# Atten4Vis/LW-DETR

Hardware: AMD Instinct MI355X
Metric: images/sec (higher is better)
Workload: dtype fp16; 1 GPU; LW-DETR-small inference forward + PostProcess, 640x640, batch 32/GPU, fp16, random-init weights (synthetic COCO-shaped input); global_batch=32, per_gpu_batch=32, parallelism=dp1, collective=none, launch_chains=2

## Files before the change

### lw-detr_amd/csrc/rowops.hip

```cpp
#include "common.h"

namespace {

constexpr int LN_MAX_CHUNKS = 16;

inline bool aligned16(const void* p) { return ((uintptr_t)p & 15) == 0; }

template <typename T, int NCH>
__global__ __launch_bounds__(256) void layernorm_kernel(const T* x, long ldx, const float* __restrict__ gamma,
                                                        const float* __restrict__ beta, T* out, long ldo,
                                                        long M, int C, float eps, long rows_per_batch,
                                                        long out_batch_rows, long out_row_offset,
                                                        const float* __restrict__ gamma2, const float* __restrict__ beta2,
                                                        T* __restrict__ out2, long ldo2, float eps2,
                                                        const float* __restrict__ part, int nsplit,
                                                        const float* __restrict__ pbias) {
    constexpr int EPC = 16 / (int)sizeof(T);
    typedef T VC __attribute__((ext_vector_type(EPC)));
    const int lane16 = threadIdx.x & 15;
    const long row = (long)blockIdx.x * 16 + (threadIdx.x >> 4);
    if (row >= M) return;
    const int nchunks = C / EPC;
    const T* xr = x + row * ldx;
    float v[NCH][EPC];
    float sum = 0.f;
#pragma unroll
    for (int i = 0; i < NCH; ++i) {
        const int c = lane16 + 16 * i;
        if (c < nchunks) {
            const VC t = *(const VC*)(xr + c * EPC);
#pragma unroll
            for (int e = 0; e < EPC; ++e) v[i][e] = to_f32<T>(t[e]);
            if (part) {
                float a[EPC];
#pragma unroll
                for (int e = 0; e < EPC; ++e) a[e] = pbias[c * EPC + e];
#pragma unroll 4
                for (int sidx = 0; sidx < nsplit; ++sidx) {
                    const float* pr = part + ((long)sidx * M + row) * C + c * EPC;
#pragma unroll
                    for (int e4 = 0; e4 < EPC; e4 += 4) {
                        const f32x4 q = *(const f32x4*)(pr + e4);
                        a[e4] += q[0]; a[e4 + 1] += q[1]; a[e4 + 2] += q[2]; a[e4 + 3] += q[3];
                    }
                }
#pragma unroll
                for (int e = 0; e < EPC; ++e) v[i][e] = to_f32<T>(from_f32<T>(v[i][e] + a[e]));
            }
#pragma unroll
            for (int e = 0; e < EPC; ++e) sum += v[i][e];
        }
    }
#pragma unroll
// ... 160 lines not shown
    hipStream_t st = (hipStream_t)hip_stream;
    switch (dtype) {
        case DT_F32: return launch_row_stats<float>(x, ldx, M, C, eps, stats, st);
        case DT_F16: return launch_row_stats<f16>(x, ldx, M, C, eps, stats, st);
        case DT_BF16: return launch_row_stats<bf16>(x, ldx, M, C, eps, stats, st);
        default: return LWDETR_ERR_UNSUPPORTED;
    }
}

extern "C" int lwdetr_layernorm(const void* x, long ldx, const float* gamma, const float* beta, void* out, long ldo,
                                long M, int C, float eps, long rows_per_batch, long out_batch_rows, long out_row_offset,
                                int dtype, void* hip_stream) {
    if (!x || !gamma || !beta || !out || M < 0 || C <= 0) return LWDETR_ERR_BAD_ARG;
    if (M == 0) return LWDETR_OK;
    hipStream_t st = (hipStream_t)hip_stream;
    switch (dtype) {
        case DT_F32: return launch_ln<float>(x, ldx, gamma, beta, out, ldo, M, C, eps, rows_per_batch, out_batch_rows, out_row_offset, st);
        case DT_F16: return launch_ln<f16>(x, ldx, gamma, beta, out, ldo, M, C, eps, rows_per_batch, out_batch_rows, out_row_offset, st);
        case DT_BF16: return launch_ln<bf16>(x, ldx, gamma, beta, out, ldo, M, C, eps, rows_per_batch, out_batch_rows, out_row_offset, st);
        default: return LWDETR_ERR_UNSUPPORTED;
    }
}

extern "C" int lwdetr_layernorm_chain(const void* x, long ldx, const float* gamma1, const float* beta1, float eps1, void* out1,
                                      long ldo1, const float* gamma2, const float* beta2, float eps2, void* out2, long ldo2,
                                      long M, int C, int dtype, void* hip_stream) {
    if (!x || !gamma1 || !beta1 || !out1 || !gamma2 || !beta2 || !out2 || M < 0 || C <= 0) return LWDETR_ERR_BAD_ARG;
    if (M == 0) return LWDETR_OK;
    hipStream_t st = (hipStream_t)hip_stream;
    switch (dtype) {
        case DT_F32: return launch_ln<float>(x, ldx, gamma1, beta1, out1, ldo1, M, C, eps1, 0, 0, 0, st, gamma2, beta2, out2, ldo2, eps2);
        case DT_F16: return launch_ln<f16>(x, ldx, gamma1, beta1, out1, ldo1, M, C, eps1, 0, 0, 0, st, gamma2, beta2, out2, ldo2, eps2);
        case DT_BF16: return launch_ln<bf16>(x, ldx, gamma1, beta1, out1, ldo1, M, C, eps1, 0, 0, 0, st, gamma2, beta2, out2, ldo2, eps2);
        default: return LWDETR_ERR_UNSUPPORTED;
    }
}

extern "C" int lwdetr_ffn_finish(const void* x, long ldx, const float* partial, int splits, const float* b2, const float* gamma1,
                                 const float* beta1, float eps1, void* out1, long ldo1, const float* gamma2, const float* beta2,
                                 float eps2, void* out2, long ldo2, long M, int C, int dtype, void* hip_stream) {
    if (!x || !partial || splits <= 0 || !b2 || !gamma1 || !beta1 || !out1 || M < 0 || C <= 0 || C % 8 != 0) return LWDETR_ERR_BAD_ARG;
    if (gamma2 && (!beta2 || !out2)) return LWDETR_ERR_BAD_ARG;
    if (M == 0) return LWDETR_OK;
    hipStream_t st = (hipStream_t)hip_stream;
    switch (dtype) {
        case DT_F16: return launch_ln<f16>(x, ldx, gamma1, beta1, out1, ldo1, M, C, eps1, 0, 0, 0, st, gamma2, beta2, out2, ldo2, eps2, partial, splits, b2);
        case DT_BF16: return launch_ln<bf16>(x, ldx, gamma1, beta1, out1, ldo1, M, C, eps1, 0, 0, 0, st, gamma2, beta2, out2, ldo2, eps2, partial, splits, b2);
        default: return LWDETR_ERR_UNSUPPORTED;
    }
}

namespace {

template <typename T>
__global__ __launch_bounds__(256) void select_gather_kernel(const T* __restrict__ om, const T* __restrict__ enc_cls, long ldc,
                                                            const float* __restrict__ props, const int64_t* __restrict__ idx,
                                                            T* __restrict__ om_sel, T* __restrict__ logits_out,
                                                            float* __restrict__ props_sel, int B, int S, int d, int nq, int ncls) {
    const long row = blockIdx.x;
    const int b = (int)(row / nq);
    const long src = (long)b * S + idx[row];
    for (int c = threadIdx.x; c < d; c += blockDim.x) om_sel[row * d + c] = om[src * d + c];
    for (int c = threadIdx.x; c < ncls; c += blockDim.x) logits_out[row * ncls + c] = enc_cls[src * ldc + c];
    if (threadIdx.x < 4) props_sel[row * 4 + threadIdx.x] = props[src * 4 + threadIdx.x];
}

template <typename T>
__global__ __launch_bounds__(256) void decoder_inputs_kernel(const T* __restrict__ enc_delta, const float* __restrict__ props_sel,
                                                             const float* __restrict__ refpoint, const float* __restrict__ vr,
                                                             int L, const T* __restrict__ query_feat,
                                                             const float* __restrict__ dim_t, T* __restrict__ enc_boxes,
                                                             float* __restrict__ ref_out, T* __restrict__ sine,
                                                             T* __restrict__ xdec, int B, int nq, int d) {
    const long row = blockIdx.x;
    const int b = (int)(row / nq), q = (int)(row - (long)b * nq);
    float dl[4], pr[4], ts[4], rp[4], rf[4];
#pragma unroll
    for (int i = 0; i < 4; ++i) { dl[i] = to_f32<T>(enc_delta[row * 4 + i]); pr[i] = props_sel[row * 4 + i]; rp[i] = refpoint[q * 4 + i]; }
    ts[0] = dl[0] * pr[2] + pr[0]; ts[1] = dl[1] * pr[3] + pr[1]; ts[2] = expf(dl[2]) * pr[2]; ts[3] = expf(dl[3]) * pr[3];
    rf[0] = rp[0] * ts[2] + ts[0]; rf[1] = rp[1] * ts[3] + ts[1]; rf[2] = expf(rp[2]) * ts[2]; rf[3] = expf(rp[3]) * ts[3];
    if (threadIdx.x < 4) { enc_boxes[row * 4 + threadIdx.x] = from_f32<T>(ts[threadIdx.x]); ref_out[row * 4 + threadIdx.x] = rf[threadIdx.x]; }
    const float vx = vr[(long)b * L * 2], vy = vr[(long)b * L * 2 + 1];
    const float pos[4] = {rf[1] * vy, rf[0] * vx, rf[2] * vx, rf[3] * vy};
    const int half = d / 2;
    for (int c = threadIdx.x; c < 2 * d; c += blockDim.x) {
        const int k = c / half, i = c - k * half;
        const float e = pos[k] * 6.283185307179586f / dim_t[i];
        sine[row * 2 * d + c] = from_f32<T>((i & 1) ? __cosf(e) : __sinf(e));
    }
    for (int c = threadIdx.x; c < d; c += blockDim.x) xdec[row * d + c] = query_feat[(long)q * d + c];
}

template <typename T>
__global__ __launch_bounds__(256) void box_reparam_kernel(const T* __restrict__ delta, const float* __restrict__ ref, long ref_rows,
                                                          T* __restrict__ out, long R) {
    const long r = (long)blockIdx.x * blockDim.x + threadIdx.x;
    if (r >= R) return;
    const float* rf = ref + (r % ref_rows) * 4;
    const float d0 = to_f32<T>(delta[r * 4]), d1 = to_f32<T>(delta[r * 4 + 1]), d2 = to_f32<T>(delta[r * 4 + 2]), d3 = to_f32<T>(delta[r * 4 + 3]);
    out[r * 4] = from_f32<T>(d0 * rf[2] + rf[0]);
    out[r * 4 + 1] = from_f32<T>(d1 * rf[3] + rf[1]);
    out[r * 4 + 2] = from_f32<T>(expf(d2) * rf[2]);
    out[r * 4 + 3] = from_f32<T>(expf(d3) * rf[3]);
}

template <typename T>
__global__ __launch_bounds__(256) void finalize_outputs_kernel(const T* __restrict__ delta, const float* __restrict__ ref, long ref_rows,
                                                               T* __restrict__ coord, long R, const T* __restrict__ logits_pad,
                                                               long ldc, int ncls, T* __restrict__ logits_out, long layer_gap) {
    const long i = (long)blockIdx.x * blockDim.x + threadIdx.x;
    if (i < R * ncls) {
        const long r = i / ncls;
        const long orow = r + (r / ref_rows) * layer_gap;
        logits_out[orow * ncls + (i - r * ncls)] = logits_pad[r * ldc + (i - r * ncls)];
    }
    if (i < R) {
        const long k = i % ref_rows;
        const float* rf = ref + k * 4;
        T* o = coord + (i + (i / ref_rows) * layer_gap) * 4;
        const float d0 = to_f32<T>(delta[i * 4]), d1 = to_f32<T>(delta[i * 4 + 1]), d2 = to_f32<T>(delta[i * 4 + 2]), d3 = to_f32<T>(delta[i * 4 + 3]);
        o[0] = from_f32<T>(d0 * rf[2] + rf[0]);
        o[1] = from_f32<T>(d1 * rf[3] + rf[1]);
        o[2] = from_f32<T>(expf(d2) * rf[2]);
        o[3] = from_f32<T>(expf(d3) * rf[3]);
    }
}

}

#define LWDETR_DISPATCH_T(dtype, CALL)                 \
    switch (dtype) {                                   \
        case DT_F32: { typedef float TT; CALL; break; } \
        case DT_F16: { typedef f16 TT; CALL; break; }   \
        case DT_BF16: { typedef bf16 TT; CALL; break; } \
        default: return LWDETR_ERR_UNSUPPORTED;        \
    }

extern "C" int lwdetr_select_gather(const void* om, const void* enc_cls, long ldc, const float* props, const int64_t* idx,
                                    void* om_sel, void* logits_out, float* props_sel, int B, int S, int d, int nq, int ncls,
                                    int dtype, void* hip_stream) {
    if (!om || !enc_cls || !props || !idx || !om_sel || !logits_out || !props_sel || B <= 0 || nq <= 0 || S <= 0 ||
        d <= 0 || ncls <= 0 || ldc < ncls) return LWDETR_ERR_BAD_ARG;
    hipStream_t st = (hipStream_t)hip_stream;
    ProfScope ps(KID_ELTWISE, 0.0, 2.0 * B * nq * (d + ncls) * 2, st);
    LWDETR_DISPATCH_T(dtype, hipLaunchKernelGGL((select_gather_kernel<TT>), dim3(B * nq), dim3(256), 0, st, (const TT*)om,
                                                (const TT*)enc_cls, ldc, props, idx, (TT*)om_sel, (TT*)logits_out, props_sel, B,
                                                S, d, nq, ncls));
    return lwdetr_check_launch();
}

extern "C" int lwdetr_decoder_inputs(const void* enc_delta, const float* props_sel, const float* refpoint, const float* valid_ratios,
                                     int L, const void* query_feat, const float* dim_t, void* enc_boxes_out, float* ref_out,
                                     void* sine_out, void* xdec_out, int B, int nq, int d, int dtype, void* hip_stream) {
    if (!enc_delta || !props_sel || !refpoint || !valid_ratios || !query_feat || !dim_t || !enc_boxes_out || !ref_out ||
        !sine_out || !xdec_out || B <= 0 || nq <= 0 || d <= 0 || d % 2 || L <= 0) return LWDETR_ERR_BAD_ARG;
    hipStream_t st = (hipStream_t)hip_stream;
    ProfScope ps(KID_ELTWISE, 0.0, 3.0 * B * nq * d * 2, st);
    LWDETR_DISPATCH_T(dtype, hipLaunchKernelGGL((decoder_inputs_kernel<TT>), dim3(B * nq), dim3(256), 0, st, (const TT*)enc_delta,
                                                props_sel, refpoint, valid_ratios, L, (const TT*)query_feat, dim_t,
                                                (TT*)enc_boxes_out, ref_out, (TT*)sine_out, (TT*)xdec_out, B, nq, d));
    return lwdetr_check_launch();
}

extern "C" int lwdetr_box_reparam(const void* delta, const float* ref, long ref_rows, void* out, long R, int dtype, void* hip_stream) {
    if (!delta || !ref || !out || R < 0 || ref_rows <= 0) return LWDETR_ERR_BAD_ARG;
    if (R == 0) return LWDETR_OK;
    hipStream_t st = (hipStream_t)hip_stream;
    ProfScope ps(KID_ELTWISE, 0.0, 0.0, st);
    LWDETR_DISPATCH_T(dtype, hipLaunchKernelGGL((box_reparam_kernel<TT>), dim3((unsigned)((R + 255) / 256)), dim3(256), 0, st,
                                                (const TT*)delta, ref, ref_rows, (TT*)out, R));
    return lwdetr_check_launch();
}

extern "C" int lwdetr_finalize_outputs(const void* delta, const float* ref, long ref_rows, void* coord_out, long R,
                                       const void* logits_pad, long ldc, int ncls, void* logits_out, long out_layer_rows, int dtype,
                                       void* hip_stream) {
    if (!delta || !ref || !coord_out || !logits_pad || !logits_out || R < 0 || ref_rows <= 0 || ncls <= 0 || ldc < ncls) return LWDETR_ERR_BAD_ARG;
    if (logits_out == logits_pad) return LWDETR_ERR_BAD_ARG;
    if (out_layer_rows == 0) out_layer_rows = ref_rows;
    if (out_layer_rows < ref_rows) return LWDETR_ERR_BAD_ARG;
    if (R == 0) return LWDETR_OK;
    hipStream_t st = (hipStream_t)hip_stream;
    ProfScope ps(KID_ELTWISE, 0.0, 0.0, st);
    const long n = R * ncls;
    LWDETR_DISPATCH_T(dtype, hipLaunchKernelGGL((finalize_outputs_kernel<TT>), dim3((unsigned)((n + 255) / 256)), dim3(256), 0, st,
                                                (const TT*)delta, ref, ref_rows, (TT*)coord_out, R, (const TT*)logits_pad, ldc, ncls,
                                                (TT*)logits_out, out_layer_rows - ref_rows));
    return lwdetr_check_launch();
}
```

### lw-detr_amd/csrc/topk.hip

```cpp
#include "common.h"

namespace {

constexpr int TK_THREADS = 1024;
constexpr int TK_MAXK = 1024;
constexpr int TK_IDX_BITS = 20;
constexpr unsigned TK_IDX_MASK = (1u << TK_IDX_BITS) - 1;

__device__ __forceinline__ unsigned fkey(float f) {
    const unsigned u = __float_as_uint(f);
    return (u & 0x80000000u) ? ~u : (u | 0x80000000u);
}
__device__ __forceinline__ float fkey_inv(unsigned k) {
    return __uint_as_float((k & 0x80000000u) ? (k ^ 0x80000000u) : ~k);
}

__device__ __forceinline__ unsigned long long tk_comp(unsigned key, int i) {
    return ((unsigned long long)key << TK_IDX_BITS) | (unsigned long long)(TK_IDX_MASK - (unsigned)i);
}

struct TopkShared {
    unsigned hist[2048];
    unsigned long long sel[TK_MAXK];
    unsigned rank[TK_MAXK];
    unsigned bstar, above, cnt, nsel;
};

template <typename T, bool CACHE>
__device__ void topk_block(const T* __restrict__ x, int N, int K, TopkShared& sh, unsigned* __restrict__ keys) {
    const int tid = threadIdx.x;
    unsigned long long prefix = 0;
    unsigned rem = (unsigned)K;
    unsigned long long thr = 0;
    int top = 32 + TK_IDX_BITS;
    bool first = true;
    while (true) {
        const int bits = top > 30 ? 11 : 10;
        const int shift = top - bits;
        const unsigned nb = 1u << bits;
        for (int i = tid; i < 2048; i += TK_THREADS) sh.hist[i] = 0;
        __syncthreads();
        if (first) {
            int i = tid;
            for (; i + 3 * TK_THREADS < N; i += 4 * TK_THREADS) {
                unsigned k4[4];
#pragma unroll
                for (int u = 0; u < 4; ++u) k4[u] = fkey(to_f32<T>(x[i + u * TK_THREADS]));
#pragma unroll
                for (int u = 0; u < 4; ++u) {
                    if (CACHE) keys[i + u * TK_THREADS] = k4[u];
                    atomicAdd(&sh.hist[k4[u] >> 21], 1u);
                }
            }
            for (; i < N; i += TK_THREADS) {
                const unsigned k = fkey(to_f32<T>(x[i]));
                if (CACHE) keys[i] = k;
                atomicAdd(&sh.hist[k >> 21], 1u);
            }
        } else {
            for (int i = tid; i < N; i += TK_THREADS) {
                const unsigned long long c = tk_comp(CACHE ? keys[i] : fkey(to_f32<T>(x[i])), i);
                if ((c >> top) == prefix) atomicAdd(&sh.hist[(unsigned)(c >> shift) & (nb - 1)], 1u);
            }
        }
        first = false;
        __syncthreads();
        if (tid < 64) {
            const int per = (int)nb >> 6;
            unsigned own = 0;
            for (int j = 0; j < per; ++j) own += sh.hist[tid * per + ((j + tid) & (per - 1))];
            unsigned s = own;
#pragma unroll
            for (int o = 1; o < 64; o <<= 1) {
                const unsigned t = __shfl_down(s, o);
                if (tid + o < 64) s += t;
            }
            const unsigned excl = s - own;
            if (excl < rem && rem <= s) {
                unsigned acc = excl;
                for (int j = per - 1; j >= 0; --j) {
                    const unsigned c = sh.hist[tid * per + j];
                    if (acc + c >= rem) { sh.bstar = (unsigned)(tid * per + j); sh.above = acc; sh.cnt = c; break; }
                    acc += c;
                }
            }
        }
        __syncthreads();
        const unsigned bstar = sh.bstar, above = sh.above, cnt = sh.cnt;
        rem -= above;
        prefix = (prefix << bits) | bstar;
        top = shift;
        if (cnt == rem || top == 0) { thr = prefix << top; break; }
    }
    if (tid == 0) sh.nsel = 0;
    for (int i = tid; i < TK_MAXK; i += TK_THREADS) sh.rank[i] = 0;
    __syncthreads();
    for (int i = tid; i < N; i += TK_THREADS) {
        const unsigned long long c = tk_comp(CACHE ? keys[i] : fkey(to_f32<T>(x[i])), i);
        if (c >= thr) {
            const unsigned p = atomicAdd(&sh.nsel, 1u);
            if (p < (unsigned)K) sh.sel[p] = c;
        }
    }
    __syncthreads();
    const int parts = TK_THREADS / K > 0 ? TK_THREADS / K : 1;
    const int e = tid % K, p = tid / K;
    if (p < parts) {
        const unsigned long long mine = sh.sel[e];
        const int j0 = (int)((long)K * p / parts), j1 = (int)((long)K * (p + 1) / parts);
        unsigned r = 0;
        for (int j = j0; j < j1; ++j) r += sh.sel[j] > mine ? 1u : 0u;
        atomicAdd(&sh.rank[e], r);
    }
    __syncthreads();
}

template <typename T, bool CACHE>
__global__ __launch_bounds__(TK_THREADS) void topk_kernel(const T* __restrict__ x, int N, int K, int64_t* __restrict__ idx_out,
                                                          float* __restrict__ val_out) {
    __shared__ TopkShared sh;
    extern __shared__ unsigned tk_keys[];
    const int b = blockIdx.x;
    topk_block<T, CACHE>(x + (long)b * N, N, K, sh, tk_keys);
    const int tid = threadIdx.x;
    if (tid < K) {
        const unsigned long long c = sh.sel[tid];
        const unsigned r = sh.rank[tid];
        idx_out[(long)b * K + r] = (int64_t)(TK_IDX_MASK - (unsigned)(c & TK_IDX_MASK));
        if (val_out) val_out[(long)b * K + r] = fkey_inv((unsigned)(c >> TK_IDX_BITS));
    }
}

template <typename T, bool CACHE>
__global__ __launch_bounds__(TK_THREADS) void postprocess_kernel(const T* __restrict__ logits, const T* __restrict__ boxes,
                                                                 const float* __restrict__ sizes, int nq, int ncls, int K,
                                                                 float* __restrict__ scores, int64_t* __restrict__ labels,
                                                                 float* __restrict__ out_boxes, float* __restrict__ packed) {
    __shared__ TopkShared sh;
    extern __shared__ unsigned tk_keys[];
    const int b = blockIdx.x;
    const int N = nq * ncls;
    topk_block<T, CACHE>(logits + (long)b * N, N, K, sh, tk_keys);
    const int tid = threadIdx.x;
    if (tid < K) {
        const unsigned long long c = sh.sel[tid];
        const long o = (long)b * K + sh.rank[tid];
        const int i = (int)(TK_IDX_MASK - (unsigned)(c & TK_IDX_MASK));
        const int q = i / ncls;
        const float v = fkey_inv((unsigned)(c >> TK_IDX_BITS));
        const float score = to_f32<T>(from_f32<T>(1.f / (1.f + expf(-v))));
        const T* bx = boxes + ((long)b * nq + q) * 4;
        const float cx = to_f32<T>(bx[0]), cy = to_f32<T>(bx[1]);
        const float w = fmaxf(to_f32<T>(bx[2]), 0.f), h = fmaxf(to_f32<T>(bx[3]), 0.f);
        const float ih = sizes[b * 2], iw = sizes[b * 2 + 1];
        const float x0 = to_f32<T>(from_f32<T>(cx - 0.5f * w)) * iw, y0 = to_f32<T>(from_f32<T>(cy - 0.5f * h)) * ih;
        const float x1 = to_f32<T>(from_f32<T>(cx + 0.5f * w)) * iw, y1 = to_f32<T>(from_f32<T>(cy + 0.5f * h)) * ih;
        if (packed) {
            float* pr = packed + o * 6;
            pr[0] = score; pr[1] = (float)(i - q * ncls); pr[2] = x0; pr[3] = y0; pr[4] = x1; pr[5] = y1;
        } else {
            scores[o] = score;
            labels[o] = (int64_t)(i - q * ncls);
            out_boxes[o * 4 + 0] = x0; out_boxes[o * 4 + 1] = y0; out_boxes[o * 4 + 2] = x1; out_boxes[o * 4 + 3] = y1;
        }
    }
}

template <typename T>
__global__ __launch_bounds__(256) void rowmax_kernel(const T* __restrict__ x, long ld, long rows, int ncols, float* __restrict__ out) {
    constexpr int EPC = 4;
    typedef T VC __attribute__((ext_vector_type(EPC)));
    const int lane16 = threadIdx.x & 15;
    const long row = (long)blockIdx.x * 16 + (threadIdx.x >> 4);
    float m = -INFINITY;
    if (row < rows) {
        const T* xr = x + row * ld;
        const int full = ncols / EPC;
        for (int c = lane16; c < full; c += 16) {
            const VC t = *(const VC*)(xr + c * EPC);
#pragma unroll
            for (int e = 0; e < EPC; ++e) m = fmaxf(m, to_f32<T>(t[e]));
        }
        for (int c = full * EPC + lane16; c < ncols; c += 16) m = fmaxf(m, to_f32<T>(xr[c]));
    }
#pragma unroll
    for (int o = 8; o >= 1; o >>= 1) m = fmaxf(m, __shfl_xor(m, o));
    if (row < rows && lane16 == 0) out[row] = m;
}

}

constexpr size_t TK_CACHE_BYTES = 160 * 1024 - sizeof(TopkShared) - 256;
static bool tk_allow_lds(const void* fn) {
    static const void* done[16]; static int ndone = 0;
    for (int i = 0; i < ndone; ++i) if (done[i] == fn) return true;
    if (hipFuncSetAttribute(fn, hipFuncAttributeMaxDynamicSharedMemorySize, (int)TK_CACHE_BYTES) != hipSuccess) return false;
    if (ndone < 16) done[ndone++] = fn;
    return true;
}

#define LWDETR_DISPATCH_T(dtype, CALL)                 \
    switch (dtype) {                                   \
        case DT_F32: { typedef float TT; CALL; break; } \
        case DT_F16: { typedef f16 TT; CALL; break; }   \
        case DT_BF16: { typedef bf16 TT; CALL; break; } \
        default: return LWDETR_ERR_UNSUPPORTED;        \
    }

extern "C" int lwdetr_rowmax(const void* x, long ld, long rows, int ncols, float* out, int dtype, void* hip_stream) {
    if (!x || !out || rows < 0 || ncols <= 0 || ld < ncols) return LWDETR_ERR_BAD_ARG;
    if (rows == 0) return LWDETR_OK;
    if (ld % 4 || ((uintptr_t)x & 15)) return LWDETR_ERR_BAD_ARG;
    hipStream_t st = (hipStream_t)hip_stream;
    ProfScope ps(KID_ELTWISE, 0.0, (double)rows * ncols * (dtype == DT_F32 ? 4 : 2), st);
    LWDETR_DISPATCH_T(dtype, hipLaunchKernelGGL((rowmax_kernel<TT>), dim3((unsigned)((rows + 15) / 16)), dim3(256), 0, st,
                                                (const TT*)x, ld, rows, ncols, out));
    return lwdetr_check_launch();
}

extern "C" int lwdetr_topk(const void* x, int B, int N, int K, int64_t* idx_out, float* val_out, int dtype, void* hip_stream) {
    if (!x || !idx_out || B < 0 || K <= 0 || K > N || K > TK_MAXK || N > (int)TK_IDX_MASK) return LWDETR_ERR_BAD_ARG;
    if (B == 0) return LWDETR_OK;
    hipStream_t st = (hipStream_t)hip_stream;
    ProfScope ps(KID_ELTWISE, 0.0, (double)B * N * (dtype == DT_F32 ? 4 : 2), st);
    const bool cache = (size_t)N * 4 <= TK_CACHE_BYTES;
    LWDETR_DISPATCH_T(dtype, {
        if (cache) {
            if (!tk_allow_lds((const void*)topk_kernel<TT, true>)) return LWDETR_ERR_LAUNCH;
            hipLaunchKernelGGL((topk_kernel<TT, true>), dim3(B), dim3(TK_THREADS), (size_t)N * 4, st, (const TT*)x, N, K, idx_out, val_out);
        } else {
            hipLaunchKernelGGL((topk_kernel<TT, false>), dim3(B), dim3(TK_THREADS), 0, st, (const TT*)x, N, K, idx_out, val_out);
        }
    });
    return lwdetr_check_launch();
}

static int postprocess_impl(const void* logits, const void* boxes, const float* target_sizes, int B, int nq, int ncls, int K,
                                  float* scores, int64_t* labels, float* out_boxes, float* packed, int dtype, void* hip_stream) {
    if (!logits || !boxes || !target_sizes || B < 0 || nq <= 0 || ncls <= 0 || K <= 0 ||
        K > TK_MAXK || (long)nq * ncls > (long)TK_IDX_MASK || K > nq * ncls)
        return LWDETR_ERR_BAD_ARG;
    if (B == 0) return LWDETR_OK;
    hipStream_t st = (hipStream_t)hip_stream;
    ProfScope ps(KID_ELTWISE, 0.0, (double)B * nq * ncls * (dtype == DT_F32 ? 4 : 2), st);
    const size_t kb = (size_t)nq * ncls * 4;
    const bool cache = kb <= TK_CACHE_BYTES;
    LWDETR_DISPATCH_T(dtype, {
        if (cache) {
            if (!tk_allow_lds((const void*)postprocess_kernel<TT, true>)) return LWDETR_ERR_LAUNCH;
            hipLaunchKernelGGL((postprocess_kernel<TT, true>), dim3(B), dim3(TK_THREADS), kb, st, (const TT*)logits, (const TT*)boxes,
                               target_sizes, nq, ncls, K, scores, labels, out_boxes, packed);
        } else {
            hipLaunchKernelGGL((postprocess_kernel<TT, false>), dim3(B), dim3(TK_THREADS), 0, st, (const TT*)logits, (const TT*)boxes,
                               target_sizes, nq, ncls, K, scores, labels, out_boxes, packed);
        }
    });
    return lwdetr_check_launch();
}

extern "C" int lwdetr_postprocess(const void* logits, const void* boxes, const float* target_sizes, int B, int nq, int ncls, int K,
                                  float* scores, int64_t* labels, float* out_boxes, int dtype, void* hip_stream) {
    if (!scores || !labels || !out_boxes) return LWDETR_ERR_BAD_ARG;
    return postprocess_impl(logits, boxes, target_sizes, B, nq, ncls, K, scores, labels, out_boxes, nullptr, dtype, hip_stream);
}

extern "C" int lwdetr_postprocess_packed(const void* logits, const void* boxes, const float* target_sizes, int B, int nq, int ncls,
                                         int K, float* packed, int dtype, void* hip_stream) {
    if (!packed) return LWDETR_ERR_BAD_ARG;
    return postprocess_impl(logits, boxes, target_sizes, B, nq, ncls, K, nullptr, nullptr, nullptr, packed, dtype, hip_stream);
}
```

Measured before the change: 14120 images/sec.

## Rework top-k radix select with range-compressed keys and vectorize decoder glue kernels

Rewrites the block-wide top-k used by two-stage proposal selection and PostProcess. It uses vectorized 16-byte loads, computes key min/max to compress the composite key, adds a candidate queue and suffix-sum histogram, picks a 512-thread variant for small N, and computes output ranks directly. The select_gather and decoder_inputs kernels now process four rows per block with one wavefront per row and 16-byte vector copies, replacing one 256-thread block per row. This targets the latency of the small serial selection kernels and the low-utilization glue kernels, at the cost of much more complex top-k code and extra LDS use. Optional timing instrumentation is included but compiled out by default.

Result: faster. 14370 images/sec, median of 6 (+1.8%).

```diff
diff --git a/lw-detr_amd/csrc/rowops.hip b/lw-detr_amd/csrc/rowops.hip
--- a/lw-detr_amd/csrc/rowops.hip
+++ b/lw-detr_amd/csrc/rowops.hip
@@ -1,4 +1,5 @@
 #include "common.h"
+#include <type_traits>
 
 namespace {
 
@@ -265,43 +266,87 @@
 
 namespace {
 
-template <typename T>
+constexpr int GLUE_ROWS = 4;
+
+template <typename T, bool VEC>
 __global__ __launch_bounds__(256) void select_gather_kernel(const T* __restrict__ om, const T* __restrict__ enc_cls, long ldc,
                                                             const float* __restrict__ props, const int64_t* __restrict__ idx,
                                                             T* __restrict__ om_sel, T* __restrict__ logits_out,
-                                                            float* __restrict__ props_sel, int B, int S, int d, int nq, int ncls) {
-    const long row = blockIdx.x;
+                                                            float* __restrict__ props_sel, long rows, int S, int d, int nq, int ncls) {
+    typedef typename Vec<T>::v8 V8;
+    typedef typename Vec<T>::v4 V4;
+    typedef typename std::conditional<sizeof(T) == 2, V8, V4>::type V;
+    constexpr int EPV = 16 / (int)sizeof(T);
+    const int lane = threadIdx.x & 63;
+    const long row = (long)blockIdx.x * GLUE_ROWS + (threadIdx.x >> 6);
+    if (row >= rows) return;
     const int b = (int)(row / nq);
     const long src = (long)b * S + idx[row];
-    for (int c = threadIdx.x; c < d; c += blockDim.x) om_sel[row * d + c] = om[src * d + c];
-    for (int c = threadIdx.x; c < ncls; c += blockDim.x) logits_out[row * ncls + c] = enc_cls[src * ldc + c];
-    if (threadIdx.x < 4) props_sel[row * 4 + threadIdx.x] = props[src * 4 + threadIdx.x];
-}
-
-template <typename T>
+    if (VEC) {
+        const V* __restrict__ sv = (const V*)(om + src * d);
+        V* __restrict__ ov = (V*)(om_sel + row * d);
+        for (int c = lane; c < d / EPV; c += 64) ov[c] = sv[c];
+    } else {
+        for (int c = lane; c < d; c += 64) om_sel[row * d + c] = om[src * d + c];
+    }
+    for (int c = lane; c < ncls; c += 64) logits_out[row * ncls + c] = enc_cls[src * ldc + c];
+    if (lane < 4) props_sel[row * 4 + lane] = props[src * 4 + lane];
+}
+
+template <typename T, bool VEC>
 __global__ __launch_bounds__(256) void decoder_inputs_kernel(const T* __restrict__ enc_delta, const float* __restrict__ props_sel,
                                                              const float* __restrict__ refpoint, const float* __restrict__ vr,
                                                              int L, const T* __restrict__ query_feat,
                                                              const float* __restrict__ dim_t, T* __restrict__ enc_boxes,
                                                              float* __restrict__ ref_out, T* __restrict__ sine,
-                                                             T* __restrict__ xdec, int B, int nq, int d) {
-    const long row = blockIdx.x;
+                                                             T* __restrict__ xdec, long rows, int nq, int d) {
+    typedef typename Vec<T>::v8 V8;
+    typedef typename Vec<T>::v4 V4;
+    typedef typename std::conditional<sizeof(T) == 2, V8, V4>::type V;
+    constexpr int EPV = 16 / (int)sizeof(T);
+    const int lane = threadIdx.x & 63;
+    const long row = (long)blockIdx.x * GLUE_ROWS + (threadIdx.x >> 6);
+    if (row >= rows) return;
     const int b = (int)(row / nq), q = (int)(row - (long)b * nq);
     float dl[4], pr[4], ts[4], rp[4], rf[4];
 #pragma unroll
     for (int i = 0; i < 4; ++i) { dl[i] = to_f32<T>(enc_delta[row * 4 + i]); pr[i] = props_sel[row * 4 + i]; rp[i] = refpoint[q * 4 + i]; }
     ts[0] = dl[0] * pr[2] + pr[0]; ts[1] = dl[1] * pr[3] + pr[1]; ts[2] = expf(dl[2]) * pr[2]; ts[3] = expf(dl[3]) * pr[3];
     rf[0] = rp[0] * ts[2] + ts[0]; rf[1] = rp[1] * ts[3] + ts[1]; rf[2] = expf(rp[2]) * ts[2]; rf[3] = expf(rp[3]) * ts[3];
-    if (threadIdx.x < 4) { enc_boxes[row * 4 + threadIdx.x] = from_f32<T>(ts[threadIdx.x]); ref_out[row * 4 + threadIdx.x] = rf[threadIdx.x]; }
+    if (lane < 4) {
+        const float t = lane == 0 ? ts[0] : lane == 1 ? ts[1] : lane == 2 ? ts[2] : ts[3];
+        const float r = lane == 0 ? rf[0] : lane == 1 ? rf[1] : lane == 2 ? rf[2] : rf[3];
+        enc_boxes[row * 4 + lane] = from_f32<T>(t);
+        ref_out[row * 4 + lane] = r;
+    }
     const float vx = vr[(long)b * L * 2], vy = vr[(long)b * L * 2 + 1];
-    const float pos[4] = {rf[1] * vy, rf[0] * vx, rf[2] * vx, rf[3] * vy};
+    const float p0 = rf[1] * vy, p1 = rf[0] * vx, p2 = rf[2] * vx, p3 = rf[3] * vy;
     const int half = d / 2;
-    for (int c = threadIdx.x; c < 2 * d; c += blockDim.x) {
-        const int k = c / half, i = c - k * half;
-        const float e = pos[k] * 6.283185307179586f / dim_t[i];
-        sine[row * 2 * d + c] = from_f32<T>((i & 1) ? __cosf(e) : __sinf(e));
-    }
-    for (int c = threadIdx.x; c < d; c += blockDim.x) xdec[row * d + c] = query_feat[(long)q * d + c];
+    if (VEC) {
+        V* __restrict__ sv = (V*)(sine + row * 2 * d);
+        for (int ch = lane; ch < 2 * d / EPV; ch += 64) {
+            const int c0 = ch * EPV, k = c0 / half, i0 = c0 - k * half;
+            const float pk = k == 0 ? p0 : k == 1 ? p1 : k == 2 ? p2 : p3;
+            V o;
+#pragma unroll
+            for (int u = 0; u < EPV; ++u) {
+                const float e = pk * 6.283185307179586f / dim_t[i0 + u];
+                o[u] = from_f32<T>((u & 1) ? __cosf(e) : __sinf(e));
+            }
+            sv[ch] = o;
+        }
+        const V* __restrict__ qv = (const V*)(query_feat + (long)q * d);
+        V* __restrict__ xv = (V*)(xdec + row * d);
+        for (int c = lane; c < d / EPV; c += 64) xv[c] = qv[c];
+    } else {
+        for (int c = lane; c < 2 * d; c += 64) {
+            const int k = c / half, i = c - k * half;
+            const float pk = k == 0 ? p0 : k == 1 ? p1 : k == 2 ? p2 : p3;
+            const float e = pk * 6.283185307179586f / dim_t[i];
+            sine[row * 2 * d + c] = from_f32<T>((i & 1) ? __cosf(e) : __sinf(e));
+        }
+        for (int c = lane; c < d; c += 64) xdec[row * d + c] = query_feat[(long)q * d + c];
+    }
 }
 
 template <typename T>
@@ -356,9 +401,15 @@
         d <= 0 || ncls <= 0 || ldc < ncls) return LWDETR_ERR_BAD_ARG;
     hipStream_t st = (hipStream_t)hip_stream;
     ProfScope ps(KID_ELTWISE, 0.0, 2.0 * B * nq * (d + ncls) * 2, st);
-    LWDETR_DISPATCH_T(dtype, hipLaunchKernelGGL((select_gather_kernel<TT>), dim3(B * nq), dim3(256), 0, st, (const TT*)om,
-                                                (const TT*)enc_cls, ldc, props, idx, (TT*)om_sel, (TT*)logits_out, props_sel, B,
-                                                S, d, nq, ncls));
+    const long rows = (long)B * nq;
+    const dim3 grid((unsigned)((rows + GLUE_ROWS - 1) / GLUE_ROWS));
+    const int epv = dtype == DT_F32 ? 4 : 8;
+    const bool vec = d % epv == 0 && !(((uintptr_t)om | (uintptr_t)om_sel) & 15);
+#define GLUE_LAUNCH(VEC)                                                                                                          \
+    hipLaunchKernelGGL((select_gather_kernel<TT, VEC>), grid, dim3(64 * GLUE_ROWS), 0, st, (const TT*)om, (const TT*)enc_cls, ldc, \
+                       props, idx, (TT*)om_sel, (TT*)logits_out, props_sel, rows, S, d, nq, ncls)
+    LWDETR_DISPATCH_T(dtype, { if (vec) GLUE_LAUNCH(true); else GLUE_LAUNCH(false); });
+#undef GLUE_LAUNCH
     return lwdetr_check_launch();
 }
 
@@ -369,9 +420,16 @@
         !sine_out || !xdec_out || B <= 0 || nq <= 0 || d <= 0 || d % 2 || L <= 0) return LWDETR_ERR_BAD_ARG;
     hipStream_t st = (hipStream_t)hip_stream;
     ProfScope ps(KID_ELTWISE, 0.0, 3.0 * B * nq * d * 2, st);
-    LWDETR_DISPATCH_T(dtype, hipLaunchKernelGGL((decoder_inputs_kernel<TT>), dim3(B * nq), dim3(256), 0, st, (const TT*)enc_delta,
-                                                props_sel, refpoint, valid_ratios, L, (const TT*)query_feat, dim_t,
-                                                (TT*)enc_boxes_out, ref_out, (TT*)sine_out, (TT*)xdec_out, B, nq, d));
+    const long rows = (long)B * nq;
+    const dim3 grid((unsigned)((rows + GLUE_ROWS - 1) / GLUE_ROWS));
+    const int epv = dtype == DT_F32 ? 4 : 8;
+    const bool vec = (d / 2) % epv == 0 && !(((uintptr_t)query_feat | (uintptr_t)sine_out | (uintptr_t)xdec_out) & 15);
+#define GLUE_LAUNCH(VEC)                                                                                                               \
+    hipLaunchKernelGGL((decoder_inputs_kernel<TT, VEC>), grid, dim3(64 * GLUE_ROWS), 0, st, (const TT*)enc_delta, props_sel, refpoint, \
+                       valid_ratios, L, (const TT*)query_feat, dim_t, (TT*)enc_boxes_out, ref_out, (TT*)sine_out, (TT*)xdec_out, rows, \
+                       nq, d)
+    LWDETR_DISPATCH_T(dtype, { if (vec) GLUE_LAUNCH(true); else GLUE_LAUNCH(false); });
+#undef GLUE_LAUNCH
     return lwdetr_check_launch();
 }
 
diff --git a/lw-detr_amd/csrc/topk.hip b/lw-detr_amd/csrc/topk.hip
--- a/lw-detr_amd/csrc/topk.hip
+++ b/lw-detr_amd/csrc/topk.hip
@@ -1,11 +1,27 @@
 #include "common.h"
+#include <type_traits>
+
+#ifdef LWDETR_TK_TIMING
+__device__ unsigned long long g_tk_timing[16];
+#define TK_TS(i) do { if (blockIdx.x == 0 && threadIdx.x == 0) g_tk_timing[i] = __builtin_amdgcn_s_memrealtime(); } while (0)
+extern "C" int lwdetr_debug_tk_timing(unsigned long long* out) {
+    return hipMemcpyFromSymbol(out, HIP_SYMBOL(g_tk_timing), sizeof(g_tk_timing)) == hipSuccess ? 0 : 1;
+}
+#else
+#define TK_TS(i) do {} while (0)
+#endif
 
 namespace {
 
-constexpr int TK_THREADS = 1024;
 constexpr int TK_MAXK = 1024;
 constexpr int TK_IDX_BITS = 20;
 constexpr unsigned TK_IDX_MASK = (1u << TK_IDX_BITS) - 1;
+constexpr int TK_BINS = 2048;
+constexpr int TK_DIGIT = 11;
+constexpr int TK_QUEUE = 128;
+constexpr int TK_CAND = 512;
+constexpr int TK_SMALL_THREADS = 512, TK_LARGE_THREADS = 1024;
+constexpr int TK_SMALL_N = 4096;
 
 __device__ __forceinline__ unsigned fkey(float f) {
     const unsigned u = __float_as_uint(f);
@@ -15,144 +31,362 @@
     return __uint_as_float((k & 0x80000000u) ? (k ^ 0x80000000u) : ~k);
 }
 
-__device__ __forceinline__ unsigned long long tk_comp(unsigned key, int i) {
-    return ((unsigned long long)key << TK_IDX_BITS) | (unsigned long long)(TK_IDX_MASK - (unsigned)i);
-}
-
-struct TopkShared {
-    unsigned hist[2048];
+template <typename T> struct TkVec { typedef typename Vec<T>::v8 type; };
+template <> struct TkVec<float> { typedef f32x4 type; };
+
+struct alignas(32) TopkShared {
+    unsigned hist[TK_BINS];
+    unsigned sfx[TK_BINS];
     unsigned long long sel[TK_MAXK];
-    unsigned rank[TK_MAXK];
+    unsigned long long cand[TK_CAND];
+    unsigned long long queue[16][TK_QUEUE];
+    unsigned wtot[16], wmin[16], wmax[16];
     unsigned bstar, above, cnt, nsel;
 };
 
-template <typename T, bool CACHE>
-__device__ void topk_block(const T* __restrict__ x, int N, int K, TopkShared& sh, unsigned* __restrict__ keys) {
+struct TkCode {
+    unsigned kmin, idxmask, bstar1;
+    int nb, sh1;
+    __device__ __forceinline__ unsigned long long comp(unsigned key, int i) const {
+        return ((unsigned long long)(key - kmin) << nb) | (unsigned long long)(idxmask - (unsigned)i);
+    }
+    __device__ __forceinline__ int index(unsigned long long c) const { return (int)(idxmask - ((unsigned)c & idxmask)); }
+    __device__ __forceinline__ float value(unsigned long long c) const { return fkey_inv((unsigned)(c >> nb) + kmin); }
+};
+
+template <typename T>
+__device__ __forceinline__ int tk_head(const T* x, int N) {
+    const int head = (int)(((16u - (unsigned)((uintptr_t)x & 15)) & 15u) / sizeof(T));
+    return head < N ? head : N;
+}
+__device__ __forceinline__ int tk_pad(int head) { return (4 - (head & 3)) & 3; }
+
+template <int NE> using TkN = std::integral_constant<int, NE>;
+template <typename F>
+struct TkEach {
+    F f;
+    template <int NE> __device__ __forceinline__ void operator()(TkN<NE>, const unsigned* k, int i0) const {
+#pragma unroll
+        for (int e = 0; e < NE; ++e) f(k[e], i0 + e);
+    }
+};
+template <typename F> __device__ __forceinline__ TkEach<F> tk_each(F f) { return TkEach<F>{f}; }
+
+template <typename T, int THREADS, typename F>
+__device__ __forceinline__ void tk_for_global(const T* __restrict__ x, int N, F f) {
+    typedef typename TkVec<T>::type VT;
+    constexpr int EPV = 16 / (int)sizeof(T);
     const int tid = threadIdx.x;
-    unsigned long long prefix = 0;
-    unsigned rem = (unsigned)K;
-    unsigned long long thr = 0;
-    int top = 32 + TK_IDX_BITS;
-    bool first = true;
-    while (true) {
-        const int bits = top > 30 ? 11 : 10;
-        const int shift = top - bits;
-        const unsigned nb = 1u << bits;
-        for (int i = tid; i < 2048; i += TK_THREADS) sh.hist[i] = 0;
-        __syncthreads();
-        if (first) {
-            int i = tid;
-            for (; i + 3 * TK_THREADS < N; i += 4 * TK_THREADS) {
-                unsigned k4[4];
-#pragma unroll
-                for (int u = 0; u < 4; ++u) k4[u] = fkey(to_f32<T>(x[i + u * TK_THREADS]));
-#pragma unroll
-                for (int u = 0; u < 4; ++u) {
-                    if (CACHE) keys[i + u * TK_THREADS] = k4[u];
-                    atomicAdd(&sh.hist[k4[u] >> 21], 1u);
+    const int head = tk_head(x, N);
+    const int nvec = (N - head) / EPV;
+    const int tail = head + nvec * EPV;
+    const bool has_h = tid < head, has_t = tail + tid < N;
+    T hv = T(0), tv = T(0);
+    if (has_h) hv = x[tid];
+    if (has_t) tv = x[tail + tid];
+    const VT* __restrict__ xv = (const VT*)(x + head);
+    for (int v0 = tid; v0 < nvec; v0 += 4 * THREADS) {
+        VT r[4];
+#pragma unroll
+        for (int u = 0; u < 4; ++u)
+            if (v0 + u * THREADS < nvec) r[u] = xv[v0 + u * THREADS];
+#pragma unroll
+        for (int u = 0; u < 4; ++u)
+            if (v0 + u * THREADS < nvec) {
+                unsigned k[EPV];
+#pragma unroll
+                for (int e = 0; e < EPV; ++e) k[e] = fkey(to_f32<T>(r[u][e]));
+                f(TkN<EPV>(), k, head + (v0 + u * THREADS) * EPV);
+            }
+    }
+    if (has_h) { const unsigned k = fkey(to_f32<T>(hv)); f(TkN<1>(), &k, tid); }
+    if (has_t) { const unsigned k = fkey(to_f32<T>(tv)); f(TkN<1>(), &k, tail + tid); }
+}
+
+template <int THREADS, typename F>
+__device__ __forceinline__ void tk_for_cached(const unsigned* __restrict__ keys, int pad, int N, F f) {
+    const uint4* __restrict__ k4 = (const uint4*)keys;
+    const int end = pad + N;
+    const int qa = (pad + 3) >> 2, qb = end >> 2;
+    for (int q = qa + (int)threadIdx.x; q < qb; q += THREADS) {
+        const uint4 v = k4[q];
+        const unsigned k[4] = {v.x, v.y, v.z, v.w};
+        f(TkN<4>(), k, q * 4 - pad);
+    }
+    if (threadIdx.x < 8) {
+        const int t = threadIdx.x;
+        const int w = t < 4 ? pad + t : 4 * (qb > qa ? qb : qa) + (t - 4);
+        if (w < end && (t >= 4 || w < 4 * qa)) { const unsigned k = keys[w]; f(TkN<1>(), &k, w - pad); }
+    }
+}
+
+template <typename T, bool CACHE, int THREADS, typename F>
+__device__ __forceinline__ void tk_for_keys(const T* __restrict__ x, const unsigned* __restrict__ keys, int pad, int N, F f) {
+    if (CACHE) tk_for_cached<THREADS>(keys, pad, N, f);
+    else tk_for_global<T, THREADS>(x, N, f);
+}
+
+template <typename T, bool CACHE, int THREADS>
+__device__ __forceinline__ void tk_load(const T* __restrict__ x, int N, unsigned* __restrict__ keys, int pad, unsigned& kmin, unsigned& kmax) {
+    typedef typename TkVec<T>::type VT;
+    constexpr int EPV = 16 / (int)sizeof(T);
+    const int tid = threadIdx.x;
+    const int head = tk_head(x, N);
+    const int nvec = (N - head) / EPV;
+    const int tail = head + nvec * EPV;
+    const bool has_h = tid < head, has_t = tail + tid < N;
+    T hv = T(0), tv = T(0);
+    if (has_h) hv = x[tid];
+    if (has_t) tv = x[tail + tid];
+    const VT* __restrict__ xv = (const VT*)(x + head);
+    for (int v0 = tid; v0 < nvec; v0 += 4 * THREADS) {
+        VT r[4];
+#pragma unroll
+        for (int u = 0; u < 4; ++u)
+            if (v0 + u * THREADS < nvec) r[u] = xv[v0 + u * THREADS];
+#pragma unroll
+        for (int u = 0; u < 4; ++u)
+            if (v0 + u * THREADS < nvec) {
+                unsigned k[EPV];
+#pragma unroll
+                for (int e = 0; e < EPV; ++e) {
+                    k[e] = fkey(to_f32<T>(r[u][e]));
+                    kmin = k[e] < kmin ? k[e] : kmin;
+                    kmax = k[e] > kmax ? k[e] : kmax;
+                }
+                if (CACHE) {
+                    uint4* dst = (uint4*)(keys + pad + head + (v0 + u * THREADS) * EPV);
+#pragma unroll
+                    for (int e = 0; e < EPV; e += 4) dst[e >> 2] = make_uint4(k[e], k[e + 1], k[e + 2], k[e + 3]);
                 }
             }
-            for (; i < N; i += TK_THREADS) {
-                const unsigned k = fkey(to_f32<T>(x[i]));
-                if (CACHE) keys[i] = k;
-                atomicAdd(&sh.hist[k >> 21], 1u);
+    }
+    if (has_h) {
+        const unsigned k = fkey(to_f32<T>(hv));
+        if (CACHE) keys[pad + tid] = k;
+        kmin = k < kmin ? k : kmin; kmax = k > kmax ? k : kmax;
+    }
+    if (has_t) {
+        const unsigned k = fkey(to_f32<T>(tv));
+        if (CACHE) keys[pad + tail + tid] = k;
+        kmin = k < kmin ? k : kmin; kmax = k > kmax ? k : kmax;
+    }
+}
+
+template <int THREADS, bool SFX>
+__device__ __forceinline__ void tk_scan(TopkShared& sh, unsigned rem, unsigned& bstar, unsigned& above, unsigned& cnt) {
+    constexpr int PER = TK_BINS / THREADS, NW = THREADS / 64;
+    typedef unsigned BinV __attribute__((ext_vector_type(PER)));
+    const int tid = threadIdx.x, lane = tid & 63, wave = tid >> 6;
+    BinV* hv = (BinV*)sh.hist;
+    const BinV cv = hv[tid];
+    hv[tid] = BinV(0);
+    unsigned own = 0;
+#pragma unroll
+    for (int j = 0; j < PER; ++j) own += cv[j];
+    unsigned s = own;
+#pragma unroll
+    for (int o = 1; o < 64; o <<= 1) {
+        const unsigned t = __shfl_down(s, o);
+        if (lane + o < 64) s += t;
+    }
+    if (lane == 0) sh.wtot[wave] = s;
+    __syncthreads();
+    unsigned excl = s - own;
+    for (int w = wave + 1; w < NW; ++w) excl += sh.wtot[w];
+    if (SFX) {
+        BinV sv;
+        unsigned acc = excl;
+#pragma unroll
+        for (int j = PER - 1; j >= 0; --j) { sv[j] = acc; acc += cv[j]; }
+        ((BinV*)sh.sfx)[tid] = sv;
+    }
+    if (excl < rem && rem <= excl + own) {
+        unsigned acc = excl;
+        bool found = false;
+#pragma unroll
+        for (int j = PER - 1; j >= 0; --j) {
+            if (!found && acc + cv[j] >= rem) { sh.bstar = (unsigned)(tid * PER + j); sh.above = acc; sh.cnt = cv[j]; found = true; }
+            acc += cv[j];
+        }
+    }
+    __syncthreads();
+    bstar = sh.bstar; above = sh.above; cnt = sh.cnt;
+}
+
+template <typename T, bool CACHE, int THREADS>
+__device__ TkCode topk_select(const T* __restrict__ x, int N, int K, TopkShared& sh, unsigned* __restrict__ keys) {
+    const int tid = threadIdx.x, lane = tid & 63;
+    TK_TS(0);
+    const int pad = tk_pad(tk_head(x, N));
+    unsigned kmin = 0xFFFFFFFFu, kmax = 0;
+    if (tid == 0) sh.nsel = 0;
+    for (int i = tid; i < TK_BINS; i += THREADS) sh.hist[i] = 0;
+    tk_load<T, CACHE, THREADS>(x, N, keys, pad, kmin, kmax);
+#pragma unroll
+    for (int o = 32; o >= 1; o >>= 1) {
+        const unsigned a = __shfl_xor(kmin, o), b = __shfl_xor(kmax, o);
+        kmin = a < kmin ? a : kmin;
+        kmax = b > kmax ? b : kmax;
+    }
+    if (lane == 0) { sh.wmin[tid >> 6] = kmin; sh.wmax[tid >> 6] = kmax; }
+    __syncthreads();
+#pragma unroll
+    for (int w = 0; w < THREADS / 64; w += 4) {
+        const uint4 a = *(const uint4*)&sh.wmin[w], b = *(const uint4*)&sh.wmax[w];
+        kmin = min(min(kmin, min(a.x, a.y)), min(a.z, a.w));
+        kmax = max(max(kmax, max(b.x, b.y)), max(b.z, b.w));
+    }
+    TK_TS(1);
+    TkCode code;
+    code.kmin = kmin;
+    const unsigned range = kmax - kmin;
+    code.nb = N > 1 ? 32 - __builtin_clz((unsigned)(N - 1)) : 0;
+    code.idxmask = (1u << code.nb) - 1u;
+    const int kb = range ? 32 - __builtin_clz(range) : 0;
+    const int bits1 = kb > TK_DIGIT ? TK_DIGIT : kb;
+    const int ksh = kb - bits1;
+    code.sh1 = ksh + code.nb;
+    tk_for_keys<T, CACHE, THREADS>(x, keys, pad, N, tk_each([&](unsigned k, int i) { atomicAdd(&sh.hist[(k - kmin) >> ksh], 1u); }));
+    __syncthreads();
+    unsigned bstar, above, cnt;
+    tk_scan<THREADS, true>(sh, (unsigned)K, bstar, above, cnt);
+    code.bstar1 = bstar;
+    unsigned rem = (unsigned)K - above;
+    TK_TS(2);
+    if (cnt == rem || cnt <= (unsigned)TK_CAND) {
+        const bool whole = cnt == rem;
+        const unsigned kthr = kmin + (bstar << ksh);
+        auto place = [&](unsigned long long c) {
+            const unsigned d = (unsigned)(c >> code.sh1);
+            if (d > bstar || whole) {
+                const unsigned p = sh.sfx[d] + atomicAdd(&sh.hist[d], 1u);
+                if (p < (unsigned)TK_MAXK) sh.sel[p] = c;
+            } else {
+                const unsigned p = atomicAdd(&sh.nsel, 1u);
+                if (p < (unsigned)TK_CAND) sh.cand[p] = c;
             }
-        } else {
-            for (int i = tid; i < N; i += TK_THREADS) {
-                const unsigned long long c = tk_comp(CACHE ? keys[i] : fkey(to_f32<T>(x[i])), i);
-                if ((c >> top) == prefix) atomicAdd(&sh.hist[(unsigned)(c >> shift) & (nb - 1)], 1u);
-            }
-        }
-        first = false;
-        __syncthreads();
-        if (tid < 64) {
-            const int per = (int)nb >> 6;
-            unsigned own = 0;
-            for (int j = 0; j < per; ++j) own += sh.hist[tid * per + ((j + tid) & (per - 1))];
-            unsigned s = own;
-#pragma unroll
-            for (int o = 1; o < 64; o <<= 1) {
-                const unsigned t = __shfl_down(s, o);
-                if (tid + o < 64) s += t;
-            }
-            const unsigned excl = s - own;
-            if (excl < rem && rem <= s) {
-                unsigned acc = excl;
-                for (int j = per - 1; j >= 0; --j) {
-                    const unsigned c = sh.hist[tid * per + j];
-                    if (acc + c >= rem) { sh.bstar = (unsigned)(tid * per + j); sh.above = acc; sh.cnt = c; break; }
-                    acc += c;
+        };
+        unsigned long long* wq = sh.queue[tid >> 6];
+        unsigned wq_n = 0;
+        tk_for_keys<T, CACHE, THREADS>(x, keys, pad, N, [&](auto ne, const unsigned* k, int i0) {
+            constexpr int NE = decltype(ne)::value;
+#pragma unroll
+            for (int e = 0; e < NE; ++e) {
+                const bool hit = k[e] >= kthr;
+                if (NE == 1) {
+                    if (hit) place(code.comp(k[e], i0 + e));
+                } else {
+                    const unsigned long long m = __ballot(hit);
+                    if (m) {
+                        const unsigned pos = wq_n + (unsigned)__popcll(m & ((1ull << lane) - 1ull));
+                        if (hit) {
+                            const unsigned long long c = code.comp(k[e], i0 + e);
+                            if (pos < (unsigned)TK_QUEUE) wq[pos] = c;
+                            else place(c);
+                        }
+                        wq_n += (unsigned)__popcll(m);
+                    }
                 }
             }
+        });
+        wq_n = (unsigned)__builtin_amdgcn_readfirstlane((int)wq_n);
+        wq_n = wq_n < (unsigned)TK_QUEUE ? wq_n : (unsigned)TK_QUEUE;
+        __threadfence_block();
+        for (unsigned j = lane; j < wq_n; j += 64) place(wq[j]);
+        __syncthreads();
+        TK_TS(3);
+        if (!whole) {
+            for (unsigned i = tid; i < cnt; i += THREADS) {
+                const unsigned long long mine = sh.cand[i];
+                unsigned r = 0;
+                for (unsigned j = 0; j < cnt; ++j) r += sh.cand[j] > mine ? 1u : 0u;
+                if (r < rem) sh.sel[above + r] = mine;
+            }
+            __syncthreads();
         }
+        TK_TS(4);
+        return code;
+    }
+    int top = code.sh1;
+    unsigned long long prefix = bstar;
+    while (top > 0) {
+        const int bits = top > TK_DIGIT ? TK_DIGIT : top;
+        const int shift = top - bits;
+        const unsigned dmask = (1u << bits) - 1u;
+        tk_for_keys<T, CACHE, THREADS>(x, keys, pad, N, tk_each([&](unsigned k, int i) {
+            const unsigned long long c = code.comp(k, i);
+            if ((c >> top) == prefix) atomicAdd(&sh.hist[(unsigned)(c >> shift) & dmask], 1u);
+        }));
         __syncthreads();
-        const unsigned bstar = sh.bstar, above = sh.above, cnt = sh.cnt;
+        tk_scan<THREADS, false>(sh, rem, bstar, above, cnt);
         rem -= above;
         prefix = (prefix << bits) | bstar;
         top = shift;
-        if (cnt == rem || top == 0) { thr = prefix << top; break; }
-    }
-    if (tid == 0) sh.nsel = 0;
-    for (int i = tid; i < TK_MAXK; i += TK_THREADS) sh.rank[i] = 0;
+        if (cnt == rem) break;
+    }
+    const unsigned long long thr = prefix << top;
+    tk_for_keys<T, CACHE, THREADS>(x, keys, pad, N, tk_each([&](unsigned k, int i) {
+        const unsigned long long c = code.comp(k, i);
+        if (c >= thr) {
+            const unsigned d = (unsigned)(c >> code.sh1);
+            const unsigned p = sh.sfx[d] + atomicAdd(&sh.hist[d], 1u);
+            if (p < (unsigned)TK_MAXK) sh.sel[p] = c;
+        }
+    }));
     __syncthreads();
-    for (int i = tid; i < N; i += TK_THREADS) {
-        const unsigned long long c = tk_comp(CACHE ? keys[i] : fkey(to_f32<T>(x[i])), i);
-        if (c >= thr) {
-            const unsigned p = atomicAdd(&sh.nsel, 1u);
-            if (p < (unsigned)K) sh.sel[p] = c;
-        }
-    }
-    __syncthreads();
-    const int parts = TK_THREADS / K > 0 ? TK_THREADS / K : 1;
-    const int e = tid % K, p = tid / K;
-    if (p < parts) {
-        const unsigned long long mine = sh.sel[e];
-        const int j0 = (int)((long)K * p / parts), j1 = (int)((long)K * (p + 1) / parts);
-        unsigned r = 0;
-        for (int j = j0; j < j1; ++j) r += sh.sel[j] > mine ? 1u : 0u;
-        atomicAdd(&sh.rank[e], r);
-    }
-    __syncthreads();
-}
-
-template <typename T, bool CACHE>
-__global__ __launch_bounds__(TK_THREADS) void topk_kernel(const T* __restrict__ x, int N, int K, int64_t* __restrict__ idx_out,
-                                                          float* __restrict__ val_out) {
+    TK_TS(8);
+    return code;
+}
+
+__device__ __forceinline__ unsigned tk_rank(const TopkShared& sh, const TkCode& code, int K, unsigned long long c) {
+    const unsigned d = (unsigned)(c >> code.sh1);
+    const unsigned lo = sh.sfx[d];
+    const unsigned below = sh.sfx[d ? d - 1 : 0];
+    const unsigned hi = d == code.bstar1 ? (unsigned)K : below;
+    unsigned r = lo;
+    for (unsigned j = lo; j < hi; ++j) r += sh.sel[j] > c ? 1u : 0u;
+    return r;
+}
+
+template <typename T, bool CACHE, int THREADS>
+__global__ __launch_bounds__(THREADS) void topk_kernel(const T* __restrict__ x, int N, int K, int64_t* __restrict__ idx_out,
+                                                       float* __restrict__ val_out) {
     __shared__ TopkShared sh;
-    extern __shared__ unsigned tk_keys[];
+    extern __shared__ __attribute__((aligned(16))) unsigned tk_keys[];
     const int b = blockIdx.x;
-    topk_block<T, CACHE>(x + (long)b * N, N, K, sh, tk_keys);
-    const int tid = threadIdx.x;
-    if (tid < K) {
-        const unsigned long long c = sh.sel[tid];
-        const unsigned r = sh.rank[tid];
-        idx_out[(long)b * K + r] = (int64_t)(TK_IDX_MASK - (unsigned)(c & TK_IDX_MASK));
-        if (val_out) val_out[(long)b * K + r] = fkey_inv((unsigned)(c >> TK_IDX_BITS));
-    }
-}
-
-template <typename T, bool CACHE>
-__global__ __launch_bounds__(TK_THREADS) void postprocess_kernel(const T* __restrict__ logits, const T* __restrict__ boxes,
-                                                                 const float* __restrict__ sizes, int nq, int ncls, int K,
-                                                                 float* __restrict__ scores, int64_t* __restrict__ labels,
-                                                                 float* __restrict__ out_boxes, float* __restrict__ packed) {
+    const TkCode code = topk_select<T, CACHE, THREADS>(x + (long)b * N, N, K, sh, tk_keys);
+    for (int e = threadIdx.x; e < K; e += THREADS) {
+        const unsigned long long c = sh.sel[e];
+        const unsigned r = tk_rank(sh, code, K, c);
+        idx_out[(long)b * K + r] = (int64_t)code.index(c);
+        if (val_out) val_out[(long)b * K + r] = code.value(c);
+    }
+    TK_TS(10);
+}
+
+template <typename T, bool CACHE, int THREADS>
+__global__ __launch_bounds__(THREADS) void postprocess_kernel(const T* __restrict__ logits, const T* __restrict__ boxes,
+                                                              const float* __restrict__ sizes, int nq, int ncls, int K,
+                                                              float* __restrict__ scores, int64_t* __restrict__ labels,
+                                                              float* __restrict__ out_boxes, float* __restrict__ packed) {
     __shared__ TopkShared sh;
-    extern __shared__ unsigned tk_keys[];
+    extern __shared__ __attribute__((aligned(16))) unsigned tk_keys[];
     const int b = blockIdx.x;
     const int N = nq * ncls;
-    topk_block<T, CACHE>(logits + (long)b * N, N, K, sh, tk_keys);
-    const int tid = threadIdx.x;
-    if (tid < K) {
-        const unsigned long long c = sh.sel[tid];
-        const long o = (long)b * K + sh.rank[tid];
-        const int i = (int)(TK_IDX_MASK - (unsigned)(c & TK_IDX_MASK));
+    const TkCode code = topk_select<T, CACHE, THREADS>(logits + (long)b * N, N, K, sh, tk_keys);
+    const float ih = sizes[b * 2], iw = sizes[b * 2 + 1];
+    for (int e = threadIdx.x; e < K; e += THREADS) {
+        const unsigned long long c = sh.sel[e];
+        const int i = code.index(c);
         const int q = i / ncls;
-        const float v = fkey_inv((unsigned)(c >> TK_IDX_BITS));
+        const T* bx = boxes + ((long)b * nq + q) * 4;
+        const T b0 = bx[0], b1 = bx[1], b2 = bx[2], b3 = bx[3];
+        const long o = (long)b * K + tk_rank(sh, code, K, c);
+        const float v = code.value(c);
         const float score = to_f32<T>(from_f32<T>(1.f / (1.f + expf(-v))));
-        const T* bx = boxes + ((long)b * nq + q) * 4;
-        const float cx = to_f32<T>(bx[0]), cy = to_f32<T>(bx[1]);
-        const float w = fmaxf(to_f32<T>(bx[2]), 0.f), h = fmaxf(to_f32<T>(bx[3]), 0.f);
-        const float ih = sizes[b * 2], iw = sizes[b * 2 + 1];
+        const float cx = to_f32<T>(b0), cy = to_f32<T>(b1);
+        const float w = fmaxf(to_f32<T>(b2), 0.f), h = fmaxf(to_f32<T>(b3), 0.f);
         const float x0 = to_f32<T>(from_f32<T>(cx - 0.5f * w)) * iw, y0 = to_f32<T>(from_f32<T>(cy - 0.5f * h)) * ih;
         const float x1 = to_f32<T>(from_f32<T>(cx + 0.5f * w)) * iw, y1 = to_f32<T>(from_f32<T>(cy + 0.5f * h)) * ih;
         if (packed) {
@@ -164,6 +398,7 @@
             out_boxes[o * 4 + 0] = x0; out_boxes[o * 4 + 1] = y0; out_boxes[o * 4 + 2] = x1; out_boxes[o * 4 + 3] = y1;
         }
     }
+    TK_TS(10);
 }
 
 template <typename T>
@@ -191,10 +426,11 @@
 }
 
 constexpr size_t TK_CACHE_BYTES = 160 * 1024 - sizeof(TopkShared) - 256;
+static size_t tk_cache_alloc(size_t n) { return ((n + 3) * 4 + 15) & ~(size_t)15; }
 static bool tk_allow_lds(const void* fn) {
     static const void* done[16]; static int ndone = 0;
     for (int i = 0; i < ndone; ++i) if (done[i] == fn) return true;
-    if (hipFuncSetAttribute(fn, hipFuncAttributeMaxDynamicSharedMemorySize, (int)TK_CACHE_BYTES) != hipSuccess) return false;
+    if (hipFuncSetAttribute(fn, hipFuncAttributeMaxDynamicSharedMemorySize, (int)tk_cache_alloc(TK_CACHE_BYTES / 4)) != hipSuccess) return false;
     if (ndone < 16) done[ndone++] = fn;
     return true;
 }
@@ -224,14 +460,19 @@
     hipStream_t st = (hipStream_t)hip_stream;
     ProfScope ps(KID_ELTWISE, 0.0, (double)B * N * (dtype == DT_F32 ? 4 : 2), st);
     const bool cache = (size_t)N * 4 <= TK_CACHE_BYTES;
+    const bool small = N <= TK_SMALL_N;
+#define TK_LAUNCH(CACHE, THREADS)                                                                                                 \
+    do {                                                                                                                           \
+        if (CACHE && !tk_allow_lds((const void*)topk_kernel<TT, CACHE, THREADS>)) return LWDETR_ERR_LAUNCH;                        \
+        hipLaunchKernelGGL((topk_kernel<TT, CACHE, THREADS>), dim3(B), dim3(THREADS), CACHE ? tk_cache_alloc((size_t)N) : 0, st, \
+                           (const TT*)x, N, K, idx_out, val_out);                                                                 \
+    } while (0)
     LWDETR_DISPATCH_T(dtype, {
-        if (cache) {
-            if (!tk_allow_lds((const void*)topk_kernel<TT, true>)) return LWDETR_ERR_LAUNCH;
-            hipLaunchKernelGGL((topk_kernel<TT, true>), dim3(B), dim3(TK_THREADS), (size_t)N * 4, st, (const TT*)x, N, K, idx_out, val_out);
-        } else {
-            hipLaunchKernelGGL((topk_kernel<TT, false>), dim3(B), dim3(TK_THREADS), 0, st, (const TT*)x, N, K, idx_out, val_out);
-        }
+        if (small) TK_LAUNCH(true, TK_SMALL_THREADS);
+        else if (cache) TK_LAUNCH(true, TK_LARGE_THREADS);
+        else TK_LAUNCH(false, TK_LARGE_THREADS);
     });
+#undef TK_LAUNCH
     return lwdetr_check_launch();
 }
 
@@ -243,18 +484,21 @@
     if (B == 0) return LWDETR_OK;
     hipStream_t st = (hipStream_t)hip_stream;
     ProfScope ps(KID_ELTWISE, 0.0, (double)B * nq * ncls * (dtype == DT_F32 ? 4 : 2), st);
-    const size_t kb = (size_t)nq * ncls * 4;
-    const bool cache = kb <= TK_CACHE_BYTES;
+    const size_t n = (size_t)nq * ncls;
+    const bool cache = n * 4 <= TK_CACHE_BYTES;
+    const bool small = n <= (size_t)TK_SMALL_N;
+#define TK_LAUNCH(CACHE, THREADS)                                                                                                  \
+    do {                                                                                                                            \
+        if (CACHE && !tk_allow_lds((const void*)postprocess_kernel<TT, CACHE, THREADS>)) return LWDETR_ERR_LAUNCH;                  \
+        hipLaunchKernelGGL((postprocess_kernel<TT, CACHE, THREADS>), dim3(B), dim3(THREADS), CACHE ? tk_cache_alloc(n) : 0, st,    \
+                           (const TT*)logits, (const TT*)boxes, target_sizes, nq, ncls, K, scores, labels, out_boxes, packed);     \
+    } while (0)
     LWDETR_DISPATCH_T(dtype, {
-        if (cache) {
-            if (!tk_allow_lds((const void*)postprocess_kernel<TT, true>)) return LWDETR_ERR_LAUNCH;
-            hipLaunchKernelGGL((postprocess_kernel<TT, true>), dim3(B), dim3(TK_THREADS), kb, st, (const TT*)logits, (const TT*)boxes,
-                               target_sizes, nq, ncls, K, scores, labels, out_boxes, packed);
-        } else {
-            hipLaunchKernelGGL((postprocess_kernel<TT, false>), dim3(B), dim3(TK_THREADS), 0, st, (const TT*)logits, (const TT*)boxes,
-                               target_sizes, nq, ncls, K, scores, labels, out_boxes, packed);
-        }
+        if (small) TK_LAUNCH(true, TK_SMALL_THREADS);
+        else if (cache) TK_LAUNCH(true, TK_LARGE_THREADS);
+        else TK_LAUNCH(false, TK_LARGE_THREADS);
     });
+#undef TK_LAUNCH
     return lwdetr_check_launch();
 }
 
```
